# yandex-research/invertible-cd

Measured on AMD Instinct MI355X. Metric: 4-step iCD images/sec (SD1.5 512^2), higher is better.
Workload: dtype f16; 1 GPU; iCD-SD1.5 4-step reverse, batch=32/GPU, fp16, 64x64 latents (512x512), w-embedding gs=7, timesteps [999,779,519,259]; per_gpu_batch=32, global_batch=32, dead_uncond_rows_eliminated=True, lora_fused=True, in_flight_batches=2, parallelism=dp1

## Files before the change

### include/icd_amd.h

```cpp
#ifndef ICD_AMD_H
#define ICD_AMD_H

#include <stdint.h>

#ifdef __cplusplus
extern "C" {
#endif

typedef enum {
    ICD_OK = 0,
    ICD_ERR_INVALID_ARG = -1,
    ICD_ERR_UNSUPPORTED = -2,
    ICD_ERR_HIP = -3,
    ICD_ERR_MISSING_TENSOR = -4,
    ICD_ERR_WORKSPACE = -5,
    ICD_ERR_HOOK = -6
} icd_status;

const char* icd_last_error(void);
int icd_version(void);
const char* icd_build_sha(void);


#define ICD_GEMM_GEGLU      1
// ... 59 lines not shown
int icd_gemm_plan(const icd_gemm_desc* d, icd_gemm_plan_info* out);
int64_t icd_gemm_workspace_bytes(int32_t M, int32_t N, int32_t K);

typedef struct {
    const void* x;
    const void* w1;
    const float* b1;
    const void* w2;
    const float* b2;
    const void* resid;
    void* out;
    int32_t M, C, hidden;
    int32_t ldx, ldw1, ldw2, ldo, ldr;
    int32_t flags;
    float ln_eps;
    const float* ln_stats;
    const float* ln_colsum;
    float* out_f32;
    const void* resid_carry;
    void* out_carry;
} icd_ffn_desc;
int icd_ffn_geglu(const icd_ffn_desc* d, void* stream);

int icd_groupnorm(const void* x0, int32_t C0, const void* x1, int32_t C1, int32_t B, int32_t HW, int32_t groups,
                  const float* gamma, const float* beta, float eps, int32_t silu, void* out, float* stats_ws,
                  void* stream);
int64_t icd_groupnorm_ws_floats(int32_t B, int32_t HW, int32_t groups);
int icd_groupnorm_carry(const void* x0, int32_t C0, const void* carry0, const void* x1, int32_t C1, const void* carry1, int32_t B,
                        int32_t HW, int32_t groups, const float* gamma, const float* beta, float eps, int32_t silu, void* out, void* aux,
                        int32_t ld_aux, float* stats_ws, void* stream);
int icd_carry_expand(const void* carry, int64_t n, void* lo, void* stream);
int icd_carry_expand2(const void* carry, const void* hi, int64_t rows, int32_t C, void* out, void* stream);

int icd_groupnorm_f32_split(const float* x, int32_t C, int32_t B, int32_t HW, int32_t groups, const float* gamma, const float* beta,
                            float eps, int32_t silu, void* out_split3, float* stats_ws, void* stream);
int icd_split_cast(const float* x, int64_t rows, int32_t C, float scale, void* out_split3, void* stream);
int icd_absmax(const float* x, int64_t n, float* out, void* stream);

int icd_layernorm(const void* x, int64_t rows, int32_t C, const float* gamma, const float* beta, float eps, void* out,
                  void* stream);
int icd_layernorm_stats(const void* x, int64_t rows, int32_t C, float eps, float* stats, void* stream);

int icd_softmax_rows(const float* s, int64_t rows, int32_t cols, int32_t ld_s, float scale, void* p, int32_t ld_p,
                     void* stream);

int icd_attention_fused(const void* q, const void* k, const void* vt, void* out, int32_t B, int32_t H, int32_t Nq,
// ... 94 lines not shown

typedef struct icd_unet icd_unet;

#define ICD_HOOK_QUERY 0
#define ICD_HOOK_PROBS 1
typedef int (*icd_attn_hook)(void* user, int32_t phase, int32_t layer, int32_t is_cross, int32_t place, int64_t bh,
                             int64_t nq, int64_t nk, int64_t ld, void** probs);

int icd_unet_create(const icd_unet_config* cfg, icd_unet** out);
void icd_unet_destroy(icd_unet* u);
int icd_unet_set_tensor(icd_unet* u, const char* name, const void* ptr, int32_t dtype, int64_t numel);
int icd_unet_finalize(icd_unet* u);
int32_t icd_unet_num_attention_layers(const icd_unet* u);
#define ICD_UNET_OPT_RESIDUAL_MODE   5
#define ICD_UNET_OPT_RESIDUAL_F32    5
#define ICD_RESIDUAL_FP16  0
#define ICD_RESIDUAL_F32   1
#define ICD_RESIDUAL_CARRY 2
#define ICD_RESIDUAL_SPLIT 3
#define ICD_UNET_OPT_SPLIT_MASK      6
#define ICD_UNET_OPT_UPSAMPLE_PHASES 7
#define ICD_UNET_OPT_GEMM_TUNE       8
#define ICD_UNET_OPT_FFN_FUSION      9
#define ICD_SPLIT_GN          1
#define ICD_SPLIT_CONV1       2
#define ICD_SPLIT_SHORTCUT    4
#define ICD_SPLIT_PROJ_OUT    8
#define ICD_SPLIT_DOWN       16
#define ICD_SPLIT_SAMPLER_OUT 32
#define ICD_SPLIT_UP         64
#define ICD_SPLIT_TEMB      128
#define ICD_SPLIT_QK        256
#define ICD_SPLIT_UP_ALL    512
#define ICD_SPLIT_ALL      1023
#define ICD_SPLIT_ACCURATE 1023
#define ICD_SPLIT_DEFAULT   447
#define ICD_UNET_OPT_XATTN_FUSION    1
#define ICD_UNET_OPT_LN_INLINE_STATS 2
#define ICD_UNET_OPT_XATTN_TILE      3
#define ICD_UNET_OPT_ATTN_VALU_SCALE 4
int icd_unet_set_option(icd_unet* u, int32_t option, int32_t value);
int64_t icd_unet_workspace_bytes(const icd_unet* u, int32_t batch, int32_t H, int32_t W, int32_t n_ctx);
int64_t icd_unet_workspace_bytes_ex(const icd_unet* u, int32_t batch, int32_t H, int32_t W, int32_t n_ctx,
                                    int32_t probs_mode);

typedef struct {
// ... 93 lines not shown
```

### invertible_cd_amd/_lib.py

```python
import ctypes as C
import os

_HERE = os.path.dirname(os.path.abspath(__file__))
LIB_PATH = os.environ.get("ICD_AMD_LIB") or os.path.join(_HERE, "lib", "libicd_amd.so")

ICD_GEMM_GEGLU = 1
ICD_GEMM_OUT_F32 = 2
ICD_GEMM_OUT_TRANS = 4
ICD_GEMM_PAD_HI = 8
ICD_GEMM_RESID_F32 = 16
ICD_GEMM_LN_COMPUTE = 32
ICD_UNET_OPT_XATTN_FUSION = 1
ICD_UNET_OPT_LN_INLINE_STATS = 2
ICD_UNET_OPT_XATTN_TILE = 3
ICD_UNET_OPT_ATTN_VALU_SCALE = 4
ICD_UNET_OPT_RESIDUAL_MODE = 5
ICD_UNET_OPT_RESIDUAL_F32 = 5
ICD_UNET_OPT_SPLIT_MASK = 6
ICD_UNET_OPT_UPSAMPLE_PHASES = 7
ICD_UNET_OPT_GEMM_TUNE = 8
ICD_UNET_OPT_FFN_FUSION = 9
ICD_GEMM_TUNE_NO_PP = 0x20000000
ICD_SPLIT_GN, ICD_SPLIT_CONV1, ICD_SPLIT_SHORTCUT, ICD_SPLIT_PROJ_OUT, ICD_SPLIT_DOWN, ICD_SPLIT_SAMPLER_OUT, ICD_SPLIT_UP, ICD_SPLIT_TEMB = 1, 2, 4, 8, 16, 32, 64, 128
ICD_SPLIT_QK = 256
ICD_SPLIT_UP_ALL = 512
ICD_SPLIT_DEFAULT, ICD_SPLIT_ACCURATE, ICD_SPLIT_ALL = 447, 1023, 1023
ICD_RESIDUAL_FP16, ICD_RESIDUAL_F32, ICD_RESIDUAL_CARRY, ICD_RESIDUAL_SPLIT = 0, 1, 2, 3
ICD_ATTN_CAUSAL = 1
ICD_ATTN_Q_PRESCALED = 2
ICD_ATTN_TUNE_MODE0 = 4
ICD_HOOK_QUERY = 0
ICD_HOOK_PROBS = 1
ICD_POOL_MAX_S2, ICD_POOL_MAX_S1P1, ICD_POOL_AVG_S1P1 = 0, 1, 2


class GemmDesc(C.Structure):
    _fields_ = [
        ("a0", C.c_void_p), ("a1", C.c_void_p), ("w", C.c_void_p), ("bias", C.c_void_p), ("rowbias", C.c_void_p),
        ("resid", C.c_void_p), ("out", C.c_void_p),
        ("M", C.c_int32), ("N", C.c_int32), ("K", C.c_int32), ("Nw", C.c_int32),
        ("lda", C.c_int32), ("ldw", C.c_int32), ("ldo", C.c_int32), ("ldr", C.c_int32), ("ld_rowbias", C.c_int32),
        ("rows_per_sample", C.c_int32), ("mode", C.c_int32), ("C0", C.c_int32), ("C1", C.c_int32),
        ("Hin", C.c_int32), ("Win", C.c_int32), ("Hout", C.c_int32), ("Wout", C.c_int32), ("ksize", C.c_int32),
        ("stride", C.c_int32), ("upsample", C.c_int32), ("batch", C.c_int32), ("zdiv", C.c_int32),
        ("a_bs0", C.c_int64), ("a_bs1", C.c_int64), ("w_bs0", C.c_int64), ("w_bs1", C.c_int64),
        ("o_bs0", C.c_int64), ("o_bs1", C.c_int64), ("alpha", C.c_float), ("flags", C.c_int32),
        ("splitk_ws", C.c_void_p), ("splitk_ws_bytes", C.c_int64),
        ("ln_stats", C.c_void_p), ("ln_colsum", C.c_void_p),
        ("xattn_k", C.c_void_p), ("xattn_vt", C.c_void_p), ("xattn_nk", C.c_int32), ("xattn_ldk", C.c_int32),
        ("xattn_ldvt", C.c_int32), ("xattn_vt_bs", C.c_int64), ("xattn_scale", C.c_float),
        ("ln_eps", C.c_float),
        ("tune_group_m", C.c_int32), ("tune_xattn_tile", C.c_int32), ("debug_timeline", C.c_void_p), ("out_f32", C.c_void_p),
        ("resid_carry", C.c_void_p), ("out_carry", C.c_void_p),
        ("conv_tap_base", C.c_int32), ("conv_ktaps", C.c_int32), ("out_remap_w", C.c_int32), ("out_remap_c", C.c_int32),
    ]


class FfnDesc(C.Structure):
    _fields_ = [("x", C.c_void_p), ("w1", C.c_void_p), ("b1", C.c_void_p), ("w2", C.c_void_p), ("b2", C.c_void_p), ("resid", C.c_void_p),
                ("out", C.c_void_p), ("M", C.c_int32), ("C", C.c_int32), ("hidden", C.c_int32), ("ldx", C.c_int32), ("ldw1", C.c_int32),
                ("ldw2", C.c_int32), ("ldo", C.c_int32), ("ldr", C.c_int32), ("flags", C.c_int32), ("ln_eps", C.c_float),
                ("ln_stats", C.c_void_p), ("ln_colsum", C.c_void_p), ("out_f32", C.c_void_p), ("resid_carry", C.c_void_p),
                ("out_carry", C.c_void_p)]


class ProbsEpilogue(C.Structure):
    _fields_ = [("acc", C.c_void_p), ("edit_At", C.c_void_p), ("edit_D", C.c_void_p), ("first_cond_sample", C.c_int32),
                ("self_from_base", C.c_int32), ("first_cond_row", C.c_int64), ("edit_count", C.c_int32), ("group_count", C.c_int32)]


class GemmPlanInfo(C.Structure):
    _fields_ = [("kernel", C.c_int32), ("tile_m", C.c_int32), ("tile_n", C.c_int32), ("ksplit", C.c_int32),
                ("ln_inline", C.c_int32), ("xattn", C.c_int32), ("cfg", C.c_int32), ("group_m", C.c_int32)]


class UNetConfig(C.Structure):
    _fields_ = [
        ("in_channels", C.c_int32), ("out_channels", C.c_int32), ("num_levels", C.c_int32),
        ("block_out_channels", C.c_int32 * 4), ("down_has_attn", C.c_int32 * 4), ("up_has_attn", C.c_int32 * 4),
        ("transformer_layers", C.c_int32 * 4), ("num_heads", C.c_int32 * 4), ("layers_per_block", C.c_int32),
        ("cross_dim", C.c_int32), ("use_linear_projection", C.c_int32), ("time_cond_proj_dim", C.c_int32),
        ("addition_time_embed_dim", C.c_int32), ("add_in_dim", C.c_int32), ("norm_groups", C.c_int32),
    ]


ATTN_HOOK = C.CFUNCTYPE(C.c_int, C.c_void_p, C.c_int32, C.c_int32, C.c_int32, C.c_int32, C.c_int64, C.c_int64,
                        C.c_int64, C.c_int64, C.POINTER(C.c_void_p))

# ... 8 lines not shown
                ("flops", C.c_double), ("tile_m", C.c_int32), ("tile_n", C.c_int32), ("plan_flags", C.c_int32), ("ksplit", C.c_int32)]


PROF_KINDS = ("gemm_conv", "gemm_dense", "gemm_batched", "attn_fused", "groupnorm", "layernorm", "softmax", "misc", "xattn_fused")


class UNetIO(C.Structure):
    _fields_ = [
        ("sample", C.c_void_p), ("timesteps", C.c_void_p), ("context", C.c_void_p), ("timestep_cond", C.c_void_p),
        ("text_embeds", C.c_void_p), ("time_ids", C.c_void_p), ("eps", C.c_void_p), ("workspace", C.c_void_p),
        ("workspace_bytes", C.c_int64), ("batch", C.c_int32), ("H", C.c_int32), ("W", C.c_int32), ("n_ctx", C.c_int32),
        ("sample_is_f32", C.c_int32), ("hook", ATTN_HOOK), ("hook_user", C.c_void_p),
        ("kv_cache", C.c_void_p), ("kv_cache_bytes", C.c_int64), ("kv_cache_valid", C.c_int32),
    ]


SIGNATURES = {
    "icd_last_error": (C.c_char_p, []),
    "icd_version": (C.c_int, []),
    "icd_build_sha": (C.c_char_p, []),
    "icd_gemm": (C.c_int, [C.POINTER(GemmDesc), C.c_void_p]),
    "icd_gemm_workspace_bytes": (C.c_int64, [C.c_int32, C.c_int32, C.c_int32]),
    "icd_ffn_geglu": (C.c_int, [C.POINTER(FfnDesc), C.c_void_p]),
    "icd_groupnorm": (C.c_int, [C.c_void_p, C.c_int32, C.c_void_p, C.c_int32, C.c_int32, C.c_int32, C.c_int32,
                                C.c_void_p, C.c_void_p, C.c_float, C.c_int32, C.c_void_p, C.c_void_p, C.c_void_p]),
    "icd_groupnorm_ws_floats": (C.c_int64, [C.c_int32, C.c_int32, C.c_int32]),
    "icd_groupnorm_carry": (C.c_int, [C.c_void_p, C.c_int32, C.c_void_p, C.c_void_p, C.c_int32, C.c_void_p, C.c_int32, C.c_int32, C.c_int32,
                                      C.c_void_p, C.c_void_p, C.c_float, C.c_int32, C.c_void_p, C.c_void_p, C.c_int32, C.c_void_p, C.c_void_p]),
    "icd_carry_expand": (C.c_int, [C.c_void_p, C.c_int64, C.c_void_p, C.c_void_p]),
    "icd_sinusoid_f32": (C.c_int, [C.c_void_p, C.c_int32, C.c_int32, C.c_int32, C.c_void_p, C.c_void_p]),
    "icd_split2_act": (C.c_int, [C.c_void_p, C.c_int64, C.c_int32, C.c_int32, C.c_void_p, C.c_void_p]),
    "icd_carry_expand2": (C.c_int, [C.c_void_p, C.c_void_p, C.c_int64, C.c_int32, C.c_void_p, C.c_void_p]),
    "icd_layernorm": (C.c_int, [C.c_void_p, C.c_int64, C.c_int32, C.c_void_p, C.c_void_p, C.c_float, C.c_void_p,
                                C.c_void_p]),
    "icd_groupnorm_f32_split": (C.c_int, [C.c_void_p, C.c_int32, C.c_int32, C.c_int32, C.c_int32, C.c_void_p, C.c_void_p, C.c_float,
                                          C.c_int32, C.c_void_p, C.c_void_p, C.c_void_p]),
    "icd_absmax": (C.c_int, [C.c_void_p, C.c_int64, C.c_void_p, C.c_void_p]),
    "icd_split_cast": (C.c_int, [C.c_void_p, C.c_int64, C.c_int32, C.c_float, C.c_void_p, C.c_void_p]),
    "icd_layernorm_stats": (C.c_int, [C.c_void_p, C.c_int64, C.c_int32, C.c_float, C.c_void_p, C.c_void_p]),
    "icd_softmax_rows": (C.c_int, [C.c_void_p, C.c_int64, C.c_int32, C.c_int32, C.c_float, C.c_void_p, C.c_int32,
                                   C.c_void_p]),
    "icd_attention_fused": (C.c_int, [C.c_void_p, C.c_void_p, C.c_void_p, C.c_void_p, C.c_int32, C.c_int32, C.c_int32,
                                      C.c_int32, C.c_int32, C.c_int32, C.c_int32, C.c_int32, C.c_int32, C.c_int64,
                                      C.c_float, C.c_void_p]),
    "icd_attention_probs": (C.c_int, [C.c_void_p, C.c_void_p, C.c_void_p] + [C.c_int32] * 8 + [C.c_float, C.c_void_p]),
    "icd_attention_probs_split": (C.c_int, [C.c_void_p] * 5 + [C.c_int32] * 8 + [C.c_float, C.c_void_p]),
# ... 148 lines not shown
```

### invertible_cd_amd/build.py

```python
import os
import subprocess
import sys
from concurrent.futures import ThreadPoolExecutor

HERE = os.path.dirname(os.path.abspath(__file__))
CSRC = os.path.join(HERE, "csrc")
LIBDIR = os.path.join(HERE, "lib")
LIB = os.path.join(LIBDIR, "libicd_amd.so")
SOURCES = ["gemm.hip", "gemm_big.hip", "gemm_pp.hip", "gemm_pp320.hip", "norm.hip", "attention.hip", "attention_masked.hip", "ffn_fused.hip", "layernorm_f32.hip", "elementwise.hip", "p2p.hip", "ingest.hip", "metrics.hip", "lpips.hip", "inception.hip", "runtime.hip", "error.cpp"]
HIPCC = os.environ.get("HIPCC", "/opt/rocm/bin/hipcc")
FLAGS = ["--offload-arch=gfx950", "-O3", "-std=c++17", "-fPIC", "-Wno-unused-value"]
EXTRA_FLAGS = {"attention.hip": ["-fno-honor-nans"]}


def source_sha():
    import hashlib
    h = hashlib.sha1()
    for f in sorted(os.listdir(CSRC)):
        if f.endswith((".hip", ".h", ".inc", ".cpp")):
            h.update(open(os.path.join(CSRC, f), "rb").read())
    return h.hexdigest()[:12]


def _deps():
    hdrs = [os.path.join(CSRC, f) for f in os.listdir(CSRC) if f.endswith(".h")]
    hdrs.append(os.path.join(HERE, "..", "include", "icd_amd.h"))
    return max(os.path.getmtime(h) for h in hdrs)


def _compile(src, force, sha):
    obj = os.path.join(LIBDIR, os.path.splitext(src)[0] + ".o")
    path = os.path.join(CSRC, src)
# ... 44 lines not shown
```

### invertible_cd_amd/csrc/runtime.hip

```cpp
#include <string>
#include <unordered_map>
#include <vector>
#include <algorithm>
#include <string.h>
#include "common.h"

namespace {

struct Tensor { const void* ptr; int dtype; long long numel; };

struct ProfRec { hipEvent_t a, b; int kind; double flops, bytes; int M, N, K, aux; int tile_m, tile_n, plan_flags, ksplit; double xflops; };
bool g_prof_on = false;
unsigned g_prof_mask = 0xffffffffu;
std::vector<ProfRec> g_prof;
std::vector<hipEvent_t> g_ev_pool;

hipEvent_t prof_event() {
    if (!g_ev_pool.empty()) { hipEvent_t e = g_ev_pool.back(); g_ev_pool.pop_back(); return e; }
    hipEvent_t e;
    (void)hipEventCreate(&e);
    return e;
}
struct ProfScope {
    bool on; hipStream_t st; size_t idx;
// ... 62 lines not shown
                }
                return;
            }
    }
};

}

struct icd_unet {
    icd_unet_config cfg;
    std::unordered_map<std::string, Tensor> tensors;
    bool finalized = false;
    int n_attn = 0;
    int temb_total = 0;
    int kv_total = 0;
    int xattn_mode = 2;
    bool ln_inline = true;
    int xattn_tile = 0;
    bool attn_mode0 = false;
    int resid_mode = 3;
    int split_mask = ICD_SPLIT_DEFAULT;
    bool up_phases = true;
    int ffn_mode = 2;
    int gemm_tune = 0;
};

namespace {

struct Act { half_t* p; int C; void* aux = nullptr; };

struct Exec {
    icd_unet* u;
    const icd_unet_io* io;
    hipStream_t st;
    Arena ar;
    bool dry;
    int probs_mode;
    std::vector<std::string>* missing;
    int B, H0, W0, nctx;
    int layer = 0;
    float* gn_ws = nullptr;
    half_t* temb_all = nullptr;
    int temb_off = 0;
    half_t* k_all = nullptr;
    half_t* vt_all = nullptr;
    unsigned char* k_all_c = nullptr;
// ... 66 lines not shown
                int ldr, half_t* out, int ldo, int flags = 0, int rps = 0, const float* ln_stats = nullptr,
                const float* ln_colsum = nullptr, const void* resid_aux = nullptr, void* out_aux = nullptr) {
        icd_gemm_desc d; memset(&d, 0, sizeof(d));
        d.a0 = a; d.w = w; d.bias = bias; d.resid = resid; d.out = out;
        d.flags = flags;
        set_aux(d, resid_aux, out_aux);
        flags = d.flags;
        d.ln_stats = ln_stats; d.ln_colsum = ln_colsum;
        d.M = M; d.N = N; d.K = K; d.Nw = N; d.lda = lda; d.ldw = K; d.ldo = ldo; d.ldr = ldr;
        d.rows_per_sample = rps; d.mode = 0; d.batch = 1; d.zdiv = 1; d.alpha = 1.f; d.flags = flags;
        gemm_desc(d);
    }
    void ffn_fused(half_t* h, int M, int C, const half_t* w1, const float* b1, const float* lnsum, float* lnst, int lnc, const half_t* w2,
                   const float* b2, const half_t* resid, void* hx) {
        if (!ok() || dry) return;
        icd_ffn_desc f; memset(&f, 0, sizeof(f));
        f.x = h; f.w1 = w1; f.b1 = b1; f.w2 = w2; f.b2 = b2; f.resid = resid; f.out = h;
        f.M = M; f.C = C; f.hidden = 4 * C; f.ldx = C; f.ldw1 = C; f.ldw2 = 4 * C; f.ldo = C; f.ldr = C;
        f.flags = lnc; f.ln_stats = lnst; f.ln_colsum = lnsum;
        if (u->resid_mode == 1) { f.resid = hx; f.flags |= ICD_GEMM_RESID_F32; f.out_f32 = (float*)hx; }
        else { f.resid_carry = hx; f.out_carry = hx; }
        ProfScope ps(true, st, ICD_PROF_GEMM_DENSE, 2.0 * M * (double)C * (8.0 * C + 4.0 * C), 0.0, M, C, 4 * C, ICD_GEMM_GEGLU);
        run(icd_ffn_geglu(&f, st));
    }
    void conv(const Act& x0, const Act* x1, int Hin, int Win, int ksize, int stride, int upsample, const half_t* w, int Cout,
              const float* bias, const half_t* rowbias, int ld_rowbias, const half_t* resid, void* out, const void* resid_aux = nullptr,
              void* out_aux = nullptr, bool out_is_f32 = false, int phase = -1) {
        icd_gemm_desc d; memset(&d, 0, sizeof(d));
        const int Hu = Hin << upsample, Wu = Win << upsample;
        const int Ho = (Hu + stride - 1) / stride, Wo = (Wu + stride - 1) / stride;
        d.a0 = x0.p; d.a1 = x1 ? x1->p : nullptr; d.w = w; d.bias = bias; d.rowbias = rowbias; d.resid = resid; d.out = out;
        d.C0 = x0.C; d.C1 = x1 ? x1->C : 0;
        d.M = B * Ho * Wo; d.N = Cout; d.K = ksize * ksize * (d.C0 + d.C1); d.Nw = Cout;
        d.ldw = d.K; d.ldo = Cout; d.ldr = Cout; d.ld_rowbias = ld_rowbias; d.rows_per_sample = Ho * Wo;
        d.mode = 1; d.Hin = Hin; d.Win = Win; d.Hout = Ho; d.Wout = Wo; d.ksize = ksize; d.stride = stride; d.upsample = upsample;
        d.batch = 1; d.zdiv = 1; d.alpha = 1.f;
        if (phase >= 0) {
            const int py = phase >> 1, px = phase & 1;
            d.conv_tap_base = 3 * py + px; d.conv_ktaps = 4; d.K = 4 * (d.C0 + d.C1); d.ldw = d.K;
            d.out_remap_w = Wo; d.out_remap_c = 2 * py * Wo + px;
        }
        set_aux(d, resid_aux, out_aux);
        if (out_is_f32) d.flags |= ICD_GEMM_OUT_F32;
        gemm_desc(d);
    }
    void free_act(Act& a) { release(a.p); release(a.aux); a.p = nullptr; a.aux = nullptr; }
// ... 153 lines not shown
        gemm_desc(g);
    }

    Act transformer(const std::string& p, const Act& x, int Hh, int Ww, int depth, int heads, int place) {
        const int HW = Hh * Ww, C = x.C, d = C / heads, X = u->cfg.cross_dim;
        const long long M = (long long)B * HW;
        const int ldv_self = (HW + 7) / 8 * 8, ldv_cross = (nctx + 7) / 8 * 8;
        half_t* n = alloc<half_t>(M * C);
        groupnorm(x, nullptr, HW, Wf(p + ".norm.weight", C), Wf(p + ".norm.bias", C), 1e-6f, 0, n);
        half_t* h = alloc<half_t>(M * C);
        void* hx = alloc_aux(M * C);
        const bool tw = u->resid_mode == 1;
        linear(n, C, (int)M, C, Wh(p + ".proj_in.weight", (long long)C * C), C, Wf(p + ".proj_in.bias", C), nullptr, 0, h, C, 0, 0,
               nullptr, nullptr, nullptr, hx);
        const int lnc = u->ln_inline ? ICD_GEMM_LN_COMPUTE : 0;
        release(n);
        float* lnst = alloc<float>(M * 2);
        for (int kb = 0; kb < depth && ok(); ++kb) {
            const std::string b = p + ".transformer_blocks." + std::to_string(kb);
            ln_stats(h, M, C, lnst);
            const AttnPlan self_plan = attn_query(false, place, heads, HW, HW);
            half_t* qk = alloc<half_t>(M * 2 * C);
            void* qk_c = (self_plan.mat && split(ICD_SPLIT_QK)) ? alloc_aux(M * 2 * C) : nullptr;
            linear(h, C, (int)M, C, Wh(b + ".attn1.to_qk.weight", 2LL * C * C), 2 * C, Wf(b + ".attn1.to_qk.lnbias", 2 * C), nullptr, 0, qk,
                   2 * C, qk_c ? (lnc | ICD_GEMM_TUNE_NO_LN_INLINE) : lnc, 0, lnst, Wf(b + ".attn1.to_qk.lnsum", 2 * C), nullptr, qk_c);
            half_t* vt = alloc<half_t>((long long)B * C * ldv_self);
            linear(h, C, (int)M, C, Wh(b + ".attn1.to_v.weight", (long long)C * C), C, nullptr, nullptr, 0, vt, ldv_self,
                   ICD_GEMM_OUT_TRANS, HW, lnst, Wf(b + ".attn1.to_v.lnsum", C));
            half_t* ao = alloc<half_t>(M * C);
            attention(self_plan, false, place, qk, 2 * C, qk + C, 2 * C, vt, ldv_self, (long long)C * ldv_self, heads, HW, HW, d, ao, C,
                      qk_c, qk_c ? (const unsigned char*)qk_c + C : nullptr);
            release(qk); release(vt); release(qk_c);
            linear(ao, C, (int)M, C, Wh(b + ".attn1.to_out.0.weight", (long long)C * C), C, Wf(b + ".attn1.to_out.0.bias", C), tw ? nullptr : h, C,
                   h, C, 0, 0, nullptr, nullptr, hx, hx);
            ln_stats(h, M, C, lnst);
            const half_t* kx = k_all + kv_off;
            const half_t* vx = vt_all + (long long)kv_off * ldv_cross;
            const long long vx_bs = (long long)u->kv_total * ldv_cross;
            const AttnPlan cross_plan = attn_query(true, place, heads, HW, nctx);
            const half_t* wq = Wh(b + ".attn2.to_q.weight", (long long)C * C);
            const float* bq = Wf(b + ".attn2.to_q.lnbias", C);
            const float* sq = Wf(b + ".attn2.to_q.lnsum", C);
            const long long xa_blocks = (M / 256) * (C / 256), xa_b192 = (long long)B * ((HW + 191) / 192) * (C / 256);
            const bool xa_auto = C % 256 == 0 && xa_blocks >= 64 && xa_b192 <= 512;
            if (!cross_plan.mat && d == 64 && C % 128 == 0 && HW % 256 == 0 && nctx <= 96 && (u->xattn_mode == 1 || (u->xattn_mode == 2 && xa_auto))) {
                if (ok() && !dry) {
                    icd_gemm_desc g; memset(&g, 0, sizeof(g));
                    g.a0 = h; g.w = wq; g.bias = bq; g.out = ao;
                    g.M = (int)M; g.N = C; g.K = C; g.Nw = C; g.lda = C; g.ldw = C; g.ldo = C;
                    g.rows_per_sample = HW; g.mode = 0; g.batch = 1; g.zdiv = 1; g.alpha = 1.f;
                    g.ln_stats = lnst; g.ln_colsum = sq; g.flags = lnc;
// ... 344 lines not shown
        u->xattn_mode = value; return ICD_OK;
    case ICD_UNET_OPT_XATTN_TILE:
        ICD_CHECK_ARG(value == 0 || value == 2 || value == 4 || value == 5 || value == 6,
                      "icd_unet_set_option: ICD_UNET_OPT_XATTN_TILE takes 0, 2, 4, 5 or 6 (got %d)", value);
        u->xattn_tile = value; return ICD_OK;
    case ICD_UNET_OPT_ATTN_VALU_SCALE:
        ICD_CHECK_ARG(value == 0 || value == 1, "icd_unet_set_option: ICD_UNET_OPT_ATTN_VALU_SCALE takes 0 or 1 (got %d)", value);
        u->attn_mode0 = value != 0; return ICD_OK;
    case ICD_UNET_OPT_RESIDUAL_MODE:
        ICD_CHECK_ARG(value >= 0 && value <= 3, "icd_unet_set_option: ICD_UNET_OPT_RESIDUAL_MODE takes 0 .. 3 (got %d)", value);
        u->resid_mode = value; return ICD_OK;
    case ICD_UNET_OPT_UPSAMPLE_PHASES:
        ICD_CHECK_ARG(value == 0 || value == 1, "icd_unet_set_option: ICD_UNET_OPT_UPSAMPLE_PHASES takes 0 or 1 (got %d)", value);
        u->up_phases = value != 0; return ICD_OK;
    case ICD_UNET_OPT_SPLIT_MASK:
        ICD_CHECK_ARG(value >= 0 && value <= ICD_SPLIT_ALL, "icd_unet_set_option: ICD_UNET_OPT_SPLIT_MASK takes a mask of ICD_SPLIT_* bits (got %d)", value);
        u->split_mask = value; return ICD_OK;
    case ICD_UNET_OPT_LN_INLINE_STATS:
        ICD_CHECK_ARG(value == 0 || value == 1, "icd_unet_set_option: ICD_UNET_OPT_LN_INLINE_STATS takes 0 or 1 (got %d)", value);
        u->ln_inline = value != 0; return ICD_OK;
    case ICD_UNET_OPT_FFN_FUSION:
        ICD_CHECK_ARG(value >= 0 && value <= 2, "icd_unet_set_option: ICD_UNET_OPT_FFN_FUSION takes 0, 1 or 2 (got %d)", value);
        u->ffn_mode = value; return ICD_OK;
    case ICD_UNET_OPT_GEMM_TUNE:
        ICD_CHECK_ARG((value & ~(ICD_GEMM_TUNE_NO_PP | ICD_GEMM_TUNE_NO_BIG | ICD_GEMM_TUNE_BN256)) == 0,
                      "icd_unet_set_option: ICD_UNET_OPT_GEMM_TUNE takes ICD_GEMM_TUNE_NO_PP / _NO_BIG / _BN256 bits (got 0x%x)", value);
        u->gemm_tune = value; return ICD_OK;
    }
    icd_set_error("icd_unet_set_option: unknown option %d", option);
    return ICD_ERR_INVALID_ARG;
}

extern "C" int icd_profile_enable(int32_t enable) {
    for (auto& r : g_prof) { g_ev_pool.push_back(r.a); g_ev_pool.push_back(r.b); }
    g_prof.clear();
    g_prof_on = enable != 0;
    g_prof_mask = enable > 0 ? 0xffffffffu : (unsigned)(-enable);
    return ICD_OK;
}

extern "C" int icd_profile_read(icd_profile_row* rows, int32_t max_rows) {
    ICD_CHECK_ARG(rows && max_rows >= ICD_PROF_KINDS, "icd_profile_read: need room for %d rows", ICD_PROF_KINDS);
    for (int k = 0; k < ICD_PROF_KINDS; ++k) { rows[k].kind = k; rows[k].launches = 0; rows[k].ms = rows[k].flops = rows[k].bytes = rows[k].flops_executed = 0.0; }
    for (auto& r : g_prof) {
        float ms = 0.f;
        if (hipEventElapsedTime(&ms, r.a, r.b) != hipSuccess) { icd_set_error("icd_profile_read: events not complete (synchronise the stream first)"); return ICD_ERR_HIP; }
// ... 120 lines not shown
```

### invertible_cd_amd/unet.py

```python
import ctypes as C
import types

import torch

from . import _lib
from .ops import geglu_perm
from .unet_config import UNetConfig

PLACES = ("down", "mid", "up")


class UNetOutput:

    def __init__(self, sample):
        self.sample = sample

    def __getitem__(self, k):
        if k == "sample" or k == 0:
            return self.sample
        raise KeyError(k)

    def __iter__(self):
        return iter((self.sample,))

# ... 193 lines not shown
        self._inverting = 0
        self._auto_plain = getattr(self, "_auto_plain", None)
        self._auto_gap = getattr(self, "_auto_gap", None)
        self.kv_cache_enabled = True
        self._kv = None

    def replica(self):
        r = object.__new__(type(self))
        for k in ("_lib", "cfg", "device", "dtype", "in_channels", "config", "_packed"):
            setattr(r, k, getattr(self, k))
        r._options = {}
        r.precision = self.precision
        r._auto_plain, r._auto_gap = self._auto_plain, self._auto_gap
        r._create_handle()
        for name, value in self._options.items():
            r.set_option(name, value)
        r.precision = self.precision
        return r

    OPTIONS = {"xattn_fusion": _lib.ICD_UNET_OPT_XATTN_FUSION, "ln_inline_stats": _lib.ICD_UNET_OPT_LN_INLINE_STATS,
               "xattn_tile": _lib.ICD_UNET_OPT_XATTN_TILE, "attn_valu_scale": _lib.ICD_UNET_OPT_ATTN_VALU_SCALE,
               "residual": _lib.ICD_UNET_OPT_RESIDUAL_MODE, "residual_f32": _lib.ICD_UNET_OPT_RESIDUAL_MODE,
               "split_mask": _lib.ICD_UNET_OPT_SPLIT_MASK, "upsample_phases": _lib.ICD_UNET_OPT_UPSAMPLE_PHASES,
               "gemm_tune": _lib.ICD_UNET_OPT_GEMM_TUNE, "ffn_fusion": _lib.ICD_UNET_OPT_FFN_FUSION}

    PRECISION = {"fast": (_lib.ICD_RESIDUAL_CARRY, _lib.ICD_SPLIT_DEFAULT), "accurate": (_lib.ICD_RESIDUAL_SPLIT, _lib.ICD_SPLIT_ACCURATE),
                 "split": (_lib.ICD_RESIDUAL_SPLIT, _lib.ICD_SPLIT_DEFAULT)}

    @classmethod
    def _env_precision(cls):
        import os
        level = os.environ.get("ICD_AMD_PRECISION", "auto")
        if level != "auto" and level not in cls.PRECISION:
            raise ValueError(f"ICD_AMD_PRECISION must be one of auto, fast, split, accurate (got {level!r})")
        return level

    def set_precision(self, level):
        if level not in (None, "auto") and level not in self.PRECISION:
            raise ValueError(f"precision must be one of auto, fast, split, accurate or None (got {level!r})")
        self.precision = level
        return self

    def editing(self):
        unet = self

        class _Inv:
            def __enter__(self_):
# ... 25 lines not shown
            self.precision = "accurate"
            e_acc = self.__call__(*args, **kwargs)
            self.precision = "fast"
            e_fast = self.__call__(*args, **kwargs)
        finally:
            self.precision = saved
        a, f = (e_acc.sample if hasattr(e_acc, "sample") else e_acc[0]), (e_fast.sample if hasattr(e_fast, "sample") else e_fast[0])
        gap = float((f.float() - a.float()).norm() / a.float().norm().clamp_min(1e-30))
        self._auto_gap = gap
        self._auto_plain = "fast" if gap <= self.AUTO_ESCALATE_GAP else "accurate"
        return e_fast if self._auto_plain == "fast" else e_acc

    def set_option(self, name, value):
        _lib.check(self._lib.icd_unet_set_option(self._h, self.OPTIONS[name], int(value)), f"icd_unet_set_option({name})")
        name = {"residual_f32": "residual"}.get(name, name)
        self._options.pop(name, None)
        self._options[name] = int(value)
        if name in ("residual", "split_mask"):
            self.precision = None
            self._applied = None
            self._kv = None
            self._ws_pool.clear()
            self._ws_key = None
        if name in ("ffn_fusion", "gemm_tune"):
            self._ws_pool.clear()
            self._ws_key = None
        return self

    def named_children(self):
        return []

    def to(self, *args, **kwargs):
        for a in list(args) + list(kwargs.values()):
            if isinstance(a, torch.dtype):
                self.dtype = a
        return self

    def eval(self):
        return self

    def __del__(self):
        try:
            if getattr(self, "_h", None):
                self._lib.icd_unet_destroy(self._h)
                self._h = None
        except Exception:
            pass
# ... 147 lines not shown
```

Before: 260.9 images/sec.

## Fuse self-attention QK and V projections into one row-resident C=320 kernel

Adds a dedicated kernel for C=320 that keeps each row of the LayerNorm input in registers, streams the QK and V weights through double-buffered LDS, and writes QK row-major and V transposed in one pass. For the 64x64 self-attention blocks it replaces two separate GEMM launches, which removes one read of the activation and one kernel launch. The kernel also computes LayerNorm stats inline when asked. It is used by default only when M is at least 65536 with no QK split and default gemm tuning. The transposed V stores are scalar and strided, which could cost write bandwidth.

```diff
diff --git a/include/icd_amd.h b/include/icd_amd.h
--- a/include/icd_amd.h
+++ b/include/icd_amd.h
@@ -105,6 +105,25 @@
 } icd_ffn_desc;
 int icd_ffn_geglu(const icd_ffn_desc* d, void* stream);
 
+typedef struct {
+    const void* x;
+    const void* w0;
+    const float* bias0;
+    const float* ln_colsum0;
+    const void* w1;
+    const float* bias1;
+    const float* ln_colsum1;
+    void* out;
+    void* out_t;
+    int32_t M, C, N, n_rowmajor, rows_per_sample;
+    int32_t ldx, ldw0, ldw1, ldo, ldt;
+    int64_t out_t_bs;
+    int32_t flags;
+    float ln_eps;
+    const float* ln_stats;
+} icd_rowproj_desc;
+int icd_rowproj320(const icd_rowproj_desc* d, void* stream);
+
 int icd_groupnorm(const void* x0, int32_t C0, const void* x1, int32_t C1, int32_t B, int32_t HW, int32_t groups,
                   const float* gamma, const float* beta, float eps, int32_t silu, void* out, float* stats_ws,
                   void* stream);
@@ -245,6 +264,7 @@
 #define ICD_UNET_OPT_UPSAMPLE_PHASES 7
 #define ICD_UNET_OPT_GEMM_TUNE       8
 #define ICD_UNET_OPT_FFN_FUSION      9
+#define ICD_UNET_OPT_ROWPROJ_FUSION  10
 #define ICD_SPLIT_GN          1
 #define ICD_SPLIT_CONV1       2
 #define ICD_SPLIT_SHORTCUT    4
diff --git a/invertible_cd_amd/_lib.py b/invertible_cd_amd/_lib.py
--- a/invertible_cd_amd/_lib.py
+++ b/invertible_cd_amd/_lib.py
@@ -20,6 +20,7 @@
 ICD_UNET_OPT_UPSAMPLE_PHASES = 7
 ICD_UNET_OPT_GEMM_TUNE = 8
 ICD_UNET_OPT_FFN_FUSION = 9
+ICD_UNET_OPT_ROWPROJ_FUSION = 10
 ICD_GEMM_TUNE_NO_PP = 0x20000000
 ICD_SPLIT_GN, ICD_SPLIT_CONV1, ICD_SPLIT_SHORTCUT, ICD_SPLIT_PROJ_OUT, ICD_SPLIT_DOWN, ICD_SPLIT_SAMPLER_OUT, ICD_SPLIT_UP, ICD_SPLIT_TEMB = 1, 2, 4, 8, 16, 32, 64, 128
 ICD_SPLIT_QK = 256
@@ -64,6 +65,14 @@
                 ("out_carry", C.c_void_p)]
 
 
+class RowprojDesc(C.Structure):
+    _fields_ = [("x", C.c_void_p), ("w0", C.c_void_p), ("bias0", C.c_void_p), ("ln_colsum0", C.c_void_p), ("w1", C.c_void_p),
+                ("bias1", C.c_void_p), ("ln_colsum1", C.c_void_p), ("out", C.c_void_p), ("out_t", C.c_void_p),
+                ("M", C.c_int32), ("C", C.c_int32), ("N", C.c_int32), ("n_rowmajor", C.c_int32), ("rows_per_sample", C.c_int32),
+                ("ldx", C.c_int32), ("ldw0", C.c_int32), ("ldw1", C.c_int32), ("ldo", C.c_int32), ("ldt", C.c_int32),
+                ("out_t_bs", C.c_int64), ("flags", C.c_int32), ("ln_eps", C.c_float), ("ln_stats", C.c_void_p)]
+
+
 class ProbsEpilogue(C.Structure):
     _fields_ = [("acc", C.c_void_p), ("edit_At", C.c_void_p), ("edit_D", C.c_void_p), ("first_cond_sample", C.c_int32),
                 ("self_from_base", C.c_int32), ("first_cond_row", C.c_int64), ("edit_count", C.c_int32), ("group_count", C.c_int32)]
@@ -118,6 +127,7 @@
     "icd_gemm": (C.c_int, [C.POINTER(GemmDesc), C.c_void_p]),
     "icd_gemm_workspace_bytes": (C.c_int64, [C.c_int32, C.c_int32, C.c_int32]),
     "icd_ffn_geglu": (C.c_int, [C.POINTER(FfnDesc), C.c_void_p]),
+    "icd_rowproj320": (C.c_int, [C.POINTER(RowprojDesc), C.c_void_p]),
     "icd_groupnorm": (C.c_int, [C.c_void_p, C.c_int32, C.c_void_p, C.c_int32, C.c_int32, C.c_int32, C.c_int32,
                                 C.c_void_p, C.c_void_p, C.c_float, C.c_int32, C.c_void_p, C.c_void_p, C.c_void_p]),
     "icd_groupnorm_ws_floats": (C.c_int64, [C.c_int32, C.c_int32, C.c_int32]),
diff --git a/invertible_cd_amd/build.py b/invertible_cd_amd/build.py
--- a/invertible_cd_amd/build.py
+++ b/invertible_cd_amd/build.py
@@ -7,7 +7,7 @@
 CSRC = os.path.join(HERE, "csrc")
 LIBDIR = os.path.join(HERE, "lib")
 LIB = os.path.join(LIBDIR, "libicd_amd.so")
-SOURCES = ["gemm.hip", "gemm_big.hip", "gemm_pp.hip", "gemm_pp320.hip", "norm.hip", "attention.hip", "attention_masked.hip", "ffn_fused.hip", "layernorm_f32.hip", "elementwise.hip", "p2p.hip", "ingest.hip", "metrics.hip", "lpips.hip", "inception.hip", "runtime.hip", "error.cpp"]
+SOURCES = ["gemm.hip", "gemm_big.hip", "gemm_pp.hip", "gemm_pp320.hip", "norm.hip", "attention.hip", "attention_masked.hip", "ffn_fused.hip", "rowproj.hip", "layernorm_f32.hip", "elementwise.hip", "p2p.hip", "ingest.hip", "metrics.hip", "lpips.hip", "inception.hip", "runtime.hip", "error.cpp"]
 HIPCC = os.environ.get("HIPCC", "/opt/rocm/bin/hipcc")
 FLAGS = ["--offload-arch=gfx950", "-O3", "-std=c++17", "-fPIC", "-Wno-unused-value"]
 EXTRA_FLAGS = {"attention.hip": ["-fno-honor-nans"]}
diff --git a/invertible_cd_amd/csrc/rowproj.hip b/invertible_cd_amd/csrc/rowproj.hip
--- /dev/null
+++ b/invertible_cd_amd/csrc/rowproj.hip
@@ -0,0 +1,226 @@
+#include "attn_frag.h"
+#include "gemm_epilogue.h"
+
+namespace {
+
+constexpr int RP_C = 320;
+constexpr int RP_KS = RP_C / 16;
+constexpr int RP_CHUNK = 64;
+constexpr int RP_STAGE = RP_CHUNK * RP_C * 2;
+constexpr int RP_LDS = 2 * RP_STAGE;
+constexpr int RP_ROWS = 128;
+constexpr int RP_NMAX = 960;
+
+struct RowK {
+    const half_t* x;
+    const half_t* w0; const float* b0; const float* s0;
+    const half_t* w1; const float* b1; const float* s1;
+    const float* ln_stats; float* ln_stats_w;
+    half_t* out; half_t* out_t;
+    long long tbs;
+    int M, N, nrm, rps, ldx, ldw0, ldw1, ldo, ldt;
+    float ln_eps;
+};
+
+template <bool LN>
+__global__ __launch_bounds__(256, 2) void rowproj320_kernel(RowK a) {
+    extern __shared__ __attribute__((aligned(1024))) unsigned char smem[];
+    const int tid = threadIdx.x, l = tid & 63, lr = l & 31, lh = l >> 5;
+    const int wv = __builtin_amdgcn_readfirstlane(tid >> 6);
+    const int m0 = blockIdx.x * RP_ROWS;
+    const int nch = a.N / RP_CHUNK, nch0 = a.nrm / RP_CHUNK;
+
+    const auto rs0 = __builtin_amdgcn_make_buffer_rsrc(const_cast<half_t*>(a.w0), 0,
+                                                       (unsigned)(((long long)(a.nrm - 1) * a.ldw0 + RP_C) * 2), 0x00020000);
+    const auto rs1 = __builtin_amdgcn_make_buffer_rsrc(const_cast<half_t*>(a.w1), 0,
+                                                       (unsigned)(((long long)(a.N - a.nrm - 1) * a.ldw1 + RP_C) * 2), 0x00020000);
+    int vr[10], vc[10];
+#pragma unroll
+    for (int i = 0; i < 10; ++i) {
+        const int s = (wv * 10 + i) * 64 + l, r = s / 40, c = (s - r * 40) ^ ((r >> 1) & 7);
+        vr[i] = r * 2; vc[i] = c * 16;
+    }
+    auto issue = [&](int j, int stage) {
+        unsigned char* d = smem + stage * RP_STAGE + wv * 10 * 1024;
+        if (j < nch0) {
+            const int so = j * RP_CHUNK * a.ldw0 * 2;
+#pragma unroll
+            for (int i = 0; i < 10; ++i)
+                __builtin_amdgcn_raw_ptr_buffer_load_lds(rs0, (__attribute__((address_space(3))) void*)(d + i * 1024), 16, vr[i] * a.ldw0 + vc[i], so, 0, 0);
+        } else {
+            const int so = (j - nch0) * RP_CHUNK * a.ldw1 * 2;
+#pragma unroll
+            for (int i = 0; i < 10; ++i)
+                __builtin_amdgcn_raw_ptr_buffer_load_lds(rs1, (__attribute__((address_space(3))) void*)(d + i * 1024), 16, vr[i] * a.ldw1 + vc[i], so, 0, 0);
+        }
+    };
+    issue(0, 0);
+
+    const int row = m0 + wv * 32 + lr;
+    const bool row_ok = row < a.M;
+    f16x8 z8;
+#pragma unroll
+    for (int e = 0; e < 8; ++e) z8[e] = (half_t)0.f;
+    f16x8 xf[RP_KS];
+    {
+        const half_t* xp = a.x + (long long)(row_ok ? row : 0) * a.ldx + lh * 8;
+#pragma unroll
+        for (int ks = 0; ks < RP_KS; ++ks) xf[ks] = *reinterpret_cast<const f16x8*>(xp + ks * 16);
+        if (!row_ok)
+#pragma unroll
+            for (int ks = 0; ks < RP_KS; ++ks) xf[ks] = z8;
+    }
+#pragma unroll
+    for (int ks = 0; ks < RP_KS; ++ks) asm volatile("" : "+v"(xf[ks]));
+    float mean = 0.f, rstd = 1.f;
+    if (LN) {
+        if (a.ln_stats_w) {
+            float s = 0.f;
+#pragma unroll
+            for (int ks = 0; ks < RP_KS; ++ks)
+#pragma unroll
+                for (int e = 0; e < 8; ++e) s += (float)xf[ks][e];
+            mean = half_sum(s) * (1.f / RP_C);
+            float q = 0.f;
+#pragma unroll
+            for (int ks = 0; ks < RP_KS; ++ks)
+#pragma unroll
+                for (int e = 0; e < 8; ++e) { const float dlt = (float)xf[ks][e] - mean; q = __builtin_fmaf(dlt, dlt, q); }
+            rstd = rsqrtf(half_sum(q) * (1.f / RP_C) + a.ln_eps);
+            if (row_ok && lh == 0) *reinterpret_cast<f32x2*>(a.ln_stats_w + 2 * (long long)row) = (f32x2){mean, rstd};
+        } else {
+            const f32x2 st = row_ok ? *reinterpret_cast<const f32x2*>(a.ln_stats + 2 * (long long)row) : (f32x2){0.f, 1.f};
+            mean = st[0]; rstd = st[1];
+        }
+    }
+    half_t* orow = a.out + (long long)row * a.ldo + 8 * lh;
+    half_t* trow = nullptr;
+    if (nch0 < nch) {
+        const int b = row / a.rps;
+        trow = a.out_t + (long long)b * a.tbs + (row - b * a.rps);
+    }
+
+    const int prow = attn_key_row(lr);
+    int t1[4];
+#pragma unroll
+    for (int q = 0; q < 4; ++q) t1[q] = prow * (RP_C * 2) + (((2 * q) | lh) ^ ((prow >> 1) & 7)) * 16;
+    const f32x16 zero16 = {0.f, 0.f, 0.f, 0.f, 0.f, 0.f, 0.f, 0.f, 0.f, 0.f, 0.f, 0.f, 0.f, 0.f, 0.f, 0.f};
+
+    auto colops = [&](int j, f32x4 (&sv)[8], f32x4 (&bv)[8]) {
+        const bool seg1 = j >= nch0;
+        const int nl = (seg1 ? j - nch0 : j) * RP_CHUNK + 8 * lh;
+        const float* bp = seg1 ? a.b1 : a.b0;
+        const float* sp = seg1 ? a.s1 : a.s0;
+#pragma unroll
+        for (int i = 0; i < 8; ++i) {
+            const int c = nl + 16 * (i >> 1) + 4 * (i & 1);
+            if (LN) sv[i] = *reinterpret_cast<const f32x4*>(sp + c);
+            bv[i] = *reinterpret_cast<const f32x4*>(bp ? bp + c : icd_gemm_detail::icd_epi_zero);
+        }
+    };
+    auto chunk = [&](int j, int stage, const f32x4 (&sv)[8], const f32x4 (&bv)[8]) {
+        const unsigned char* sb = smem + stage * RP_STAGE;
+        const bool seg1 = j >= nch0;
+        const int nl = (seg1 ? j - nch0 : j) * RP_CHUNK;
+#pragma unroll
+        for (int t = 0; t < 2; ++t) {
+            f32x16 acc = zero16;
+#pragma unroll
+            for (int ks = 0; ks < RP_KS; ++ks) {
+                const f16x8 wf = *reinterpret_cast<const f16x8*>(sb + t * 32 * RP_C * 2 + t1[ks & 3] + (ks >> 2) * 128);
+                acc = __builtin_amdgcn_mfma_f32_32x32x16_f16(wf, xf[ks], acc, 0, 0, 0);
+            }
+            float v[16];
+#pragma unroll
+            for (int g = 0; g < 2; ++g)
+#pragma unroll
+                for (int e = 0; e < 8; ++e) {
+                    float x = acc[8 * g + e];
+                    if (LN) x = rstd * (x - mean * sv[4 * t + 2 * g + (e >> 2)][e & 3]);
+                    x += bv[4 * t + 2 * g + (e >> 2)][e & 3];
+                    v[8 * g + e] = x;
+                }
+            if (!seg1) {
+                if (row_ok)
+#pragma unroll
+                    for (int g = 0; g < 2; ++g) {
+                        f16x8 o;
+#pragma unroll
+                        for (int e = 0; e < 8; ++e) o[e] = (half_t)v[8 * g + e];
+                        *reinterpret_cast<f16x8*>(orow + j * RP_CHUNK + 32 * t + 16 * g) = o;
+                    }
+            } else if (row_ok) {
+                half_t* tp = trow + (long long)(nl + 32 * t + 8 * lh) * a.ldt;
+#pragma unroll
+                for (int g = 0; g < 2; ++g)
+#pragma unroll
+                    for (int e = 0; e < 8; ++e) tp[(long long)(16 * g + e) * a.ldt] = (half_t)v[8 * g + e];
+            }
+        }
+    };
+
+    for (int j = 0; j < nch; ++j) {
+        asm volatile("s_waitcnt vmcnt(0)" ::: "memory");
+        __syncthreads();
+        f32x4 sv[8], bv[8];
+        colops(j, sv, bv);
+        if (j + 1 < nch) issue(j + 1, (j + 1) & 1);
+        chunk(j, j & 1, sv, bv);
+    }
+}
+
+template <bool LN>
+int launch(const RowK& k, hipStream_t st) {
+    static std::atomic<unsigned long long> armed{0};
+    return icd_launch_lds(armed, "icd_rowproj320", rowproj320_kernel<LN>, dim3((k.M + RP_ROWS - 1) / RP_ROWS), dim3(256), RP_LDS, st, k);
+}
+
+}
+
+extern "C" int icd_rowproj320(const icd_rowproj_desc* d, void* stream) {
+    ICD_CHECK_ARG(d != nullptr, "icd_rowproj320: descriptor must be non-null");
+    ICD_CHECK_ARG(d->C == RP_C, "icd_rowproj320: C = %d: the kernel is built for C = 320", d->C);
+    ICD_CHECK_ARG(d->M > 0, "icd_rowproj320: M = %d must be positive", d->M);
+    ICD_CHECK_ARG(d->N > 0 && d->N <= RP_NMAX && d->N % RP_CHUNK == 0, "icd_rowproj320: N = %d must be a multiple of 64, at most 960", d->N);
+    ICD_CHECK_ARG(d->n_rowmajor >= 0 && d->n_rowmajor <= d->N && d->n_rowmajor % RP_CHUNK == 0,
+                  "icd_rowproj320: n_rowmajor = %d must be a multiple of 64 in [0, N]", d->n_rowmajor);
+    ICD_CHECK_ARG((d->flags & ~ICD_GEMM_LN_COMPUTE) == 0, "icd_rowproj320: flags 0x%x: only ICD_GEMM_LN_COMPUTE", d->flags);
+    const bool seg0 = d->n_rowmajor > 0, seg1 = d->n_rowmajor < d->N;
+    ICD_CHECK_ARG(d->x, "icd_rowproj320: x must be non-null");
+    ICD_CHECK_ARG(d->ldx >= RP_C && d->ldx % 8 == 0, "icd_rowproj320: ldx = %d must be a multiple of 8, >= C", d->ldx);
+    if (seg0) {
+        ICD_CHECK_ARG(d->w0 && d->out, "icd_rowproj320: w0 and out must be non-null with row-major columns");
+        ICD_CHECK_ARG(d->ldw0 >= RP_C && d->ldw0 % 8 == 0, "icd_rowproj320: ldw0 = %d must be a multiple of 8, >= C", d->ldw0);
+        ICD_CHECK_ARG(d->ldo >= d->n_rowmajor && d->ldo % 8 == 0, "icd_rowproj320: ldo = %d must be a multiple of 8, >= n_rowmajor", d->ldo);
+        ICD_CHECK_ARG((long long)d->n_rowmajor * d->ldw0 * 2 < (1ll << 31), "icd_rowproj320: ldw0 beyond 31-bit byte offsets");
+    }
+    if (seg1) {
+        ICD_CHECK_ARG(d->w1 && d->out_t, "icd_rowproj320: w1 and out_t must be non-null with transposed columns");
+        ICD_CHECK_ARG(d->ldw1 >= RP_C && d->ldw1 % 8 == 0, "icd_rowproj320: ldw1 = %d must be a multiple of 8, >= C", d->ldw1);
+        ICD_CHECK_ARG((long long)(d->N - d->n_rowmajor) * d->ldw1 * 2 < (1ll << 31), "icd_rowproj320: ldw1 beyond 31-bit byte offsets");
+        ICD_CHECK_ARG(d->rows_per_sample > 0 && d->rows_per_sample % 32 == 0 && d->M % d->rows_per_sample == 0,
+                      "icd_rowproj320: rows_per_sample = %d must be a positive multiple of 32 that divides M with transposed columns", d->rows_per_sample);
+        ICD_CHECK_ARG(d->ldt >= d->rows_per_sample && d->ldt % 8 == 0, "icd_rowproj320: ldt = %d must be a multiple of 8, >= rows_per_sample", d->ldt);
+        ICD_CHECK_ARG(d->out_t_bs >= (long long)(d->N - d->n_rowmajor) * d->ldt, "icd_rowproj320: out_t_bs smaller than one sample's transposed columns");
+    }
+    const bool ln = d->ln_stats != nullptr || (d->flags & ICD_GEMM_LN_COMPUTE);
+    ICD_CHECK_ARG(!(d->flags & ICD_GEMM_LN_COMPUTE) || d->ln_stats, "icd_rowproj320: ICD_GEMM_LN_COMPUTE stores the statistics: ln_stats must be non-null");
+    ICD_CHECK_ARG(!ln || ((!seg0 || d->ln_colsum0) && (!seg1 || d->ln_colsum1)),
+                  "icd_rowproj320: the LayerNorm fold needs ln_colsum (row sums of the gamma-scaled W) for every segment");
+    ICD_CHECK_ARG(ln || (!d->ln_colsum0 && !d->ln_colsum1), "icd_rowproj320: ln_colsum without ln_stats: give both for the LayerNorm fold, or neither");
+    const uintptr_t al16 = (uintptr_t)d->x | (uintptr_t)d->w0 | (uintptr_t)d->w1 | (uintptr_t)d->out | (uintptr_t)d->out_t | (uintptr_t)d->bias0 |
+                           (uintptr_t)d->bias1 | (uintptr_t)d->ln_colsum0 | (uintptr_t)d->ln_colsum1;
+    ICD_CHECK_ARG((al16 & 15) == 0, "icd_rowproj320: x, w0, w1, out, out_t, bias and ln_colsum must be 16-byte aligned");
+    ICD_CHECK_ARG(((uintptr_t)d->ln_stats & 7) == 0, "icd_rowproj320: ln_stats must be 8-byte aligned");
+    RowK k = {};
+    k.x = (const half_t*)d->x;
+    k.w0 = (const half_t*)d->w0; k.b0 = d->bias0; k.s0 = d->ln_colsum0;
+    k.w1 = (const half_t*)d->w1; k.b1 = d->bias1; k.s1 = d->ln_colsum1;
+    k.ln_stats = d->ln_stats; k.ln_stats_w = (d->flags & ICD_GEMM_LN_COMPUTE) ? const_cast<float*>(d->ln_stats) : nullptr;
+    k.out = (half_t*)d->out; k.out_t = (half_t*)d->out_t; k.tbs = d->out_t_bs;
+    k.M = d->M; k.N = d->N; k.nrm = d->n_rowmajor; k.rps = seg1 ? d->rows_per_sample : 1;
+    k.ldx = d->ldx; k.ldw0 = d->ldw0; k.ldw1 = d->ldw1; k.ldo = d->ldo; k.ldt = d->ldt;
+    k.ln_eps = d->ln_eps > 0.f ? d->ln_eps : 1e-5f;
+    hipStream_t st = (hipStream_t)stream;
+    return ln ? launch<true>(k, st) : launch<false>(k, st);
+}
diff --git a/invertible_cd_amd/csrc/runtime.hip b/invertible_cd_amd/csrc/runtime.hip
--- a/invertible_cd_amd/csrc/runtime.hip
+++ b/invertible_cd_amd/csrc/runtime.hip
@@ -108,6 +108,7 @@
     int split_mask = ICD_SPLIT_DEFAULT;
     bool up_phases = true;
     int ffn_mode = 2;
+    int rowproj_mode = 2;
     int gemm_tune = 0;
 };
 
@@ -220,6 +221,17 @@
         else { f.resid_carry = hx; f.out_carry = hx; }
         ProfScope ps(true, st, ICD_PROF_GEMM_DENSE, 2.0 * M * (double)C * (8.0 * C + 4.0 * C), 0.0, M, C, 4 * C, ICD_GEMM_GEGLU);
         run(icd_ffn_geglu(&f, st));
+    }
+    void qkv_fused(const half_t* h, int M, int C, int HW, const half_t* wqk, const float* bqk, const float* sqk, const half_t* wv,
+                   const float* sv, float* lnst, int lnc, half_t* qk, half_t* vt, int ldv) {
+        if (!ok() || dry) return;
+        icd_rowproj_desc r; memset(&r, 0, sizeof(r));
+        r.x = h; r.w0 = wqk; r.bias0 = bqk; r.ln_colsum0 = sqk; r.w1 = wv; r.ln_colsum1 = sv; r.out = qk; r.out_t = vt;
+        r.M = M; r.C = C; r.N = 3 * C; r.n_rowmajor = 2 * C; r.rows_per_sample = HW;
+        r.ldx = C; r.ldw0 = C; r.ldw1 = C; r.ldo = 2 * C; r.ldt = ldv; r.out_t_bs = (long long)C * ldv;
+        r.flags = lnc; r.ln_stats = lnst;
+        ProfScope ps(true, st, ICD_PROF_GEMM_DENSE, 2.0 * M * (double)C * (3.0 * C), 0.0, M, 3 * C, C, ICD_GEMM_OUT_TRANS);
+        run(icd_rowproj320(&r, st));
     }
     void conv(const Act& x0, const Act* x1, int Hin, int Win, int ksize, int stride, int upsample, const half_t* w, int Cout,
               const float* bias, const half_t* rowbias, int ld_rowbias, const half_t* resid, void* out, const void* resid_aux = nullptr,
@@ -419,11 +431,21 @@
             const AttnPlan self_plan = attn_query(false, place, heads, HW, HW);
             half_t* qk = alloc<half_t>(M * 2 * C);
             void* qk_c = (self_plan.mat && split(ICD_SPLIT_QK)) ? alloc_aux(M * 2 * C) : nullptr;
+            half_t* vt = nullptr;
+            const bool rowproj = C == 320 && HW % 128 == 0 && !qk_c && !tw &&
+                                 (u->rowproj_mode == 1 || (u->rowproj_mode == 2 && M >= 65536 && u->gemm_tune == 0));
+            if (rowproj) {
+                vt = alloc<half_t>((long long)B * C * ldv_self);
+                qkv_fused(h, (int)M, C, HW, Wh(b + ".attn1.to_qk.weight", 2LL * C * C), Wf(b + ".attn1.to_qk.lnbias", 2 * C),
+                          Wf(b + ".attn1.to_qk.lnsum", 2 * C), Wh(b + ".attn1.to_v.weight", (long long)C * C), Wf(b + ".attn1.to_v.lnsum", C),
+                          lnst, lnc, qk, vt, ldv_self);
+            } else {
             linear(h, C, (int)M, C, Wh(b + ".attn1.to_qk.weight", 2LL * C * C), 2 * C, Wf(b + ".attn1.to_qk.lnbias", 2 * C), nullptr, 0, qk,
                    2 * C, qk_c ? (lnc | ICD_GEMM_TUNE_NO_LN_INLINE) : lnc, 0, lnst, Wf(b + ".attn1.to_qk.lnsum", 2 * C), nullptr, qk_c);
-            half_t* vt = alloc<half_t>((long long)B * C * ldv_self);
+            vt = alloc<half_t>((long long)B * C * ldv_self);
             linear(h, C, (int)M, C, Wh(b + ".attn1.to_v.weight", (long long)C * C), C, nullptr, nullptr, 0, vt, ldv_self,
                    ICD_GEMM_OUT_TRANS, HW, lnst, Wf(b + ".attn1.to_v.lnsum", C));
+            }
             half_t* ao = alloc<half_t>(M * C);
             attention(self_plan, false, place, qk, 2 * C, qk + C, 2 * C, vt, ldv_self, (long long)C * ldv_self, heads, HW, HW, d, ao, C,
                       qk_c, qk_c ? (const unsigned char*)qk_c + C : nullptr);
@@ -814,6 +836,9 @@
     case ICD_UNET_OPT_FFN_FUSION:
         ICD_CHECK_ARG(value >= 0 && value <= 2, "icd_unet_set_option: ICD_UNET_OPT_FFN_FUSION takes 0, 1 or 2 (got %d)", value);
         u->ffn_mode = value; return ICD_OK;
+    case ICD_UNET_OPT_ROWPROJ_FUSION:
+        ICD_CHECK_ARG(value >= 0 && value <= 2, "icd_unet_set_option: ICD_UNET_OPT_ROWPROJ_FUSION takes 0, 1 or 2 (got %d)", value);
+        u->rowproj_mode = value; return ICD_OK;
     case ICD_UNET_OPT_GEMM_TUNE:
         ICD_CHECK_ARG((value & ~(ICD_GEMM_TUNE_NO_PP | ICD_GEMM_TUNE_NO_BIG | ICD_GEMM_TUNE_BN256)) == 0,
                       "icd_unet_set_option: ICD_UNET_OPT_GEMM_TUNE takes ICD_GEMM_TUNE_NO_PP / _NO_BIG / _BN256 bits (got 0x%x)", value);
diff --git a/invertible_cd_amd/unet.py b/invertible_cd_amd/unet.py
--- a/invertible_cd_amd/unet.py
+++ b/invertible_cd_amd/unet.py
@@ -239,7 +239,8 @@
                "xattn_tile": _lib.ICD_UNET_OPT_XATTN_TILE, "attn_valu_scale": _lib.ICD_UNET_OPT_ATTN_VALU_SCALE,
                "residual": _lib.ICD_UNET_OPT_RESIDUAL_MODE, "residual_f32": _lib.ICD_UNET_OPT_RESIDUAL_MODE,
                "split_mask": _lib.ICD_UNET_OPT_SPLIT_MASK, "upsample_phases": _lib.ICD_UNET_OPT_UPSAMPLE_PHASES,
-               "gemm_tune": _lib.ICD_UNET_OPT_GEMM_TUNE, "ffn_fusion": _lib.ICD_UNET_OPT_FFN_FUSION}
+               "gemm_tune": _lib.ICD_UNET_OPT_GEMM_TUNE, "ffn_fusion": _lib.ICD_UNET_OPT_FFN_FUSION,
+               "rowproj_fusion": _lib.ICD_UNET_OPT_ROWPROJ_FUSION}
 
     PRECISION = {"fast": (_lib.ICD_RESIDUAL_CARRY, _lib.ICD_SPLIT_DEFAULT), "accurate": (_lib.ICD_RESIDUAL_SPLIT, _lib.ICD_SPLIT_ACCURATE),
                  "split": (_lib.ICD_RESIDUAL_SPLIT, _lib.ICD_SPLIT_DEFAULT)}
@@ -311,7 +312,7 @@
             self._kv = None
             self._ws_pool.clear()
             self._ws_key = None
-        if name in ("ffn_fusion", "gemm_tune"):
+        if name in ("ffn_fusion", "rowproj_fusion", "gemm_tune"):
             self._ws_pool.clear()
             self._ws_key = None
         return self
```

After: 262.3 images/sec (median of 6 runs). Within noise of the previous version (+0.5%).
